# ArtyZe/yolo_quantization

Hardware: AMD Instinct MI355X
Metric: images/sec yolov3-tiny INT8 416x416 (higher is better)
Workload: dtype u8 x s8 -> int32 (f64 or exact-integer requant, bit-identical); 1 GPU; yolov3-tiny full net (cfg/yolov3-tiny_quant.cfg, leaky, per-channel quant), batch 64/GPU synthetic uint8 416x416, inputs resident in HBM (NCHW uint8); global_batch=64, parallelism=image-sharded x1, RCCL weight broadcast once, batches_in_flight=4, kernel_plan=throughput (kernels of which two workgroups share a CU)

## Files before the change

### yolo_quantization_amd/csrc/conv_rows16.hip

```cpp
#include "kargs.h"
#include <type_traits>

#define DBG(bit) (false)
#if defined(MI355_ABLATE)
__device__ long long g_rows16_ts[6][4096];
#define TS(k) do { if (threadIdx.x == 0 && blockIdx.x < 4096) g_rows16_ts[k][blockIdx.x] = wall_clock64(); } while (0)
extern "C" int mi355_debug_read_ts16(long long *host)
{
    return hipMemcpyFromSymbol(host, HIP_SYMBOL(g_rows16_ts), sizeof(long long) * 6 * 4096) == hipSuccess ? 0 : -5;
}
#else
#define TS(k) do { } while (0)
#endif
#define WP_DECL do { } while (0)
#define WP_START() do { } while (0)
#define WP_MARK(k) do { } while (0)
#define WP_FLUSH() do { } while (0)

#define DMA16(gsrc, ldst)                                                                               \
    __builtin_amdgcn_global_load_lds((const __attribute__((address_space(1))) void *)(gsrc),           \
                                     (__attribute__((address_space(3))) void *)(ldst), 16, 0, 0)

template <int KS, int BN> constexpr int ra16_stages() { return KS == 3 ? (BN <= 192 ? 4 : 6) : (BN <= 128 ? 4 : 3); }
template <int KS, int BN> constexpr int rb16_stages() { return KS == 3 ? 2 : ra16_stages<KS, BN>(); }
constexpr int rows16_nb_slots(int BN, int RS, int NW, int KS)
{
    const int wmin = RS * 3 / 4, halo = KS == 3 ? 1 : 0;
    const int rows = (BN - 2 + wmin) / wmin + 1 + (BN - 2 + wmin * wmin) / (wmin * wmin) + 2 * halo;
    return (rows * (RS / 16) + NW - 1) / NW;
}

__device__ __forceinline__ void row16_of_pixel(int n, int H, int W, FastDiv fd_hw, FastDiv fd_w, int &grow, int &x)
{
    const int hw = H * W;
    const int b = fd_div(n, fd_hw);
    const int r = n - b * hw;
    const int y = fd_div(r, fd_w);
    x = r - y * W;
    grow = b * (H + 1) + y + 1;
}

template <int BM, int BN, int WMW, int WNW, int RS, int KS, int NBX = 0>
__global__ __launch_bounds__(64 * WMW * WNW, (BM / WMW > 64 ? 1 : 2)) void conv_rows16_i8_kernel(const ConvArgs a)
{
    constexpr int NW = WMW * WNW, NT = 64 * NW;
    constexpr int TM = BM / WMW, TN = BN / WNW;
    constexpr int MI = TM / 16, NI = TN / 16;
    constexpr int ACH = BM / 16;
    static_assert(KS == 3 && TN % 32 == 0, "3x3 only; pixels are dealt in 32-column sub-tiles (two 16-column tiles each)");
    constexpr int DW = (NW == 8 && KS == 3) ? 4 : NW;
    constexpr int APT = (ACH + DW - 1) / DW;
    constexpr int HALO = (KS == 3) ? 1 : 0;
    constexpr int PIECEB = RS * 16;
    constexpr int CPR = RS / 16;
    constexpr int OSTR = BM + 4;
    constexpr int RA_STAGES = ra16_stages<KS, BN>();
    constexpr int RB_STAGES = rb16_stages<KS, BN>();
    constexpr int NBS = rows16_nb_slots(BN, RS, DW, KS) + NBX;
    constexpr int SPS = (NBS + 3) / 4;
    static_assert(TM % 16 == 0 && TN % 32 == 0, "wave tile: 16-row tiles, 32-column sub-tiles");

    extern __shared__ __attribute__((aligned(16))) char smem[];
    char *ldsB = smem + RA_STAGES * BM * 64;
    const int rowb = a.rowb;
    const int bbytes = a.rows_cap * rowb;
    int *ldsS = reinterpret_cast<int *>(ldsB + RB_STAGES * bbytes);
    double *ldsPM = reinterpret_cast<double *>(smem + a.lds_param_off);
    int *ldsPI = reinterpret_cast<int *>(ldsPM + 3 * BM);
    float *ldsYL = reinterpret_cast<float *>(ldsPI + 2 * BM);

    const int tid = threadIdx.x;
    const int lane = tid & 63;
    const int wave = __builtin_amdgcn_readfirstlane(tid >> 6);
    const int wm = wave / WNW, wn = wave % WNW;
    const int kq = lane >> 4, lj = lane & 15;
    const int dwave = wave & (DW - 1);
    const bool issuer = wave < DW;
    TS(0);

    int logical;
    {
        const int nb = gridDim.x, id = blockIdx.x;
        const int q = nb >> 3, r = nb & 7, xcd = id & 7, idx = id >> 3;
        logical = (xcd < r ? xcd * (q + 1) : r * (q + 1) + (xcd - r) * q) + idx;
    }
    int mtile, ntile;
    {
        const int blk = fd_div(logical, a.fd_ntper);
        const int rem = logical - blk * (a.xcd_mb * a.ntiles_n);
        ntile = fd_div(rem, a.fd_mb);
        mtile = blk * a.xcd_mb + (rem - ntile * a.xcd_mb);
    }
    const int n0 = ntile * a.tile_q + min(ntile, a.tile_r);
    const int n_end = n0 + a.tile_q + (ntile < a.tile_r ? 1 : 0);
    const int W1 = a.W + 1, hw = a.H * a.W;

    int gr0, x0;
    row16_of_pixel(n0, a.H, a.W, a.fd_hw, a.fd_w, gr0, x0);
    int gr1, x1;
    row16_of_pixel(n_end - 1, a.H, a.W, a.fd_hw, a.fd_w, gr1, x1);
    const int grow_first = gr0 - HALO;
    const int nrows = gr1 - gr0 + 1 + 2 * HALO;
    const int ndma = nrows * CPR;

    constexpr int NS = NI;
    int bbase[NS];
#pragma unroll
    for (int ns = 0; ns < NS; ++ns) {
        const int n = n0 + ((ns >> 1) * WNW + wn) * 32 + (ns & 1) * 16 + lj;
        int gr, x;
        row16_of_pixel(n < n_end ? n : n_end - 1, a.H, a.W, a.fd_hw, a.fd_w, gr, x);
        const int prow = gr - grow_first - HALO;
        const int pcol = x + 1 - HALO;
        bbase[ns] = prow * rowb + pcol * 16 + kq * PIECEB;
    }
    const int atab0 = (wm * MI) * 1024 + lane * 16;

    const unsigned lds0 = (unsigned)(size_t)(__attribute__((address_space(3))) char *)smem;
#define DMA_S(ldsdst_u32, sbase_ptr, voff_u32)                                                                   \
    asm volatile("s_mov_b32 m0, %0\n\ts_nop 0\n\tglobal_load_lds_dwordx4 %1, %2" ::"s"(ldsdst_u32), "v"(voff_u32), \
                 "s"(sbase_ptr)                                                                                  \
                 : "memory", "m0")
    constexpr int TAPS = KS * KS;
    const int rot = a.debug & 512 ? 0 : ntile - fd_div(ntile, a.fd_nch) * a.nchunks;
    const int kwrap = a.ksteps;
    int aleft = kwrap - rot * TAPS;
    const int8_t *aptr[APT];
    unsigned adst[APT];
#pragma unroll
    for (int i = 0; i < APT; ++i) {
        const int ch = min(dwave + i * DW, ACH - 1);
        aptr[i] = a.wp + ((size_t)(mtile * ACH + ch) * a.ksteps + (size_t)rot * TAPS) * 1024;
        adst[i] = lds0 + (ch << 10);
    }
    const unsigned lane16 = lane * 16;
    auto issueA_next = [&](unsigned stage_off) {
        if (DW < NW && !issuer) return;
        const bool wrap = --aleft == 0;
#pragma unroll
        for (int i = 0; i < APT; ++i) {
            DMA_S(adst[i] + stage_off, aptr[i], lane16);
            aptr[i] += wrap ? 1024 - (long)kwrap * 1024 : 1024;
        }
        if (wrap) aleft = kwrap;
    };
    const long cell0 = (long)a.in_lead + (long)grow_first * W1 - 1;
    unsigned bvoff[NBS], bdst[NBS];
#pragma unroll
    for (int i = 0; i < NBS; ++i) {
        const int j = min(dwave + i * DW, ndma - 1);
        const int r = j / CPR, cj = j - r * CPR;
        const int o = cj * 1024 + lane * 16;
        const int p = o / PIECEB, c = (o - p * PIECEB) >> 4;
        long f = cell0 + (long)r * W1 + c;
        f = f < 0 ? 0 : (f > a.in_cells - 1 ? a.in_cells - 1 : f);
        bvoff[i] = (unsigned)(f * a.in_cs + p * 16);
        bdst[i] = lds0 + RA_STAGES * BM * 64 + r * rowb + (cj << 10);
    }
    auto issueB_slots = [&](int chunk, auto lo_c, auto hi_c) {
        constexpr int LO = decltype(lo_c)::value, HI = decltype(hi_c)::value;
        if (DW < NW && !issuer) return;
        const unsigned boff = (chunk % RB_STAGES) * bbytes;
        int phys = chunk + rot;
        if (phys >= a.nchunks) phys -= a.nchunks;
        const int8_t *base = a.x + (size_t)phys * 64;
#pragma unroll
        for (int i = LO; i < HI; ++i) {
            const unsigned d = bdst[i] + boff, v = bvoff[i];
            DMA_S(d, base, v);
        }
    };
    auto issueB = [&](int chunk) { issueB_slots(chunk, std::integral_constant<int, 0>{}, std::integral_constant<int, NBS>{}); };

    TS(1);
    if constexpr (KS == 3) {
        issueB(0);
#pragma unroll
        for (int st = 0; st < RA_STAGES - 1; ++st) issueA_next(st * (BM * 64));
    } else {
#pragma unroll
        for (int st = 0; st < RA_STAGES - 1; ++st)
            if (st < a.ksteps) {
                issueB(st);
                issueA_next(st * (BM * 64));
            }
    }

    v4i acc[MI][NI];
#pragma unroll
    for (int mi = 0; mi < MI; ++mi) {
        const int4 c4 = *reinterpret_cast<const int4 *>(a.cwb + mtile * BM + wm * TM + mi * 16 + 4 * kq);
#pragma unroll
        for (int ni = 0; ni < NI; ++ni) acc[mi][ni] = v4i{c4.x, c4.y, c4.z, c4.w};
    }

    for (int i = tid; i < a.rows_cap * RS; i += NT) ldsS[i] = 0;
    if (a.yolo_out)
        for (int i = tid; i < 256; i += NT) ldsYL[i] = yolo_entry_act((float)(i - a.zp_act) * a.s_act, 0);
    for (int i = tid; i < BM; i += NT) {
        const int oc = mtile * BM + i;
        ldsPM[i] = a.mval[oc];
        ldsPM[BM + i] = a.sval[oc];
        ldsPI[i] = a.dzp[oc];
        ldsPI[BM + i] = a.bias[oc];
        ldsPM[2 * BM + i] = a.mprime[oc];
    }

    auto cell_sums = [&](const char *Bt) {
        const int ncells = nrows * RS;
        for (int id = tid; id < ncells; id += NT) {
            const int r = id / RS, c = id - r * RS;
            const char *p0 = Bt + r * rowb + c * 16;
            int t = 0;
#pragma unroll 1
            for (int p = 0; p < 4; ++p) {
                const v4i v = *reinterpret_cast<const v4i *>(p0 + p * PIECEB);
                t = __builtin_amdgcn_sdot4(v[0], 0x01010101, t, false);
                t = __builtin_amdgcn_sdot4(v[1], 0x01010101, t, false);
                t = __builtin_amdgcn_sdot4(v[2], 0x01010101, t, false);
                t = __builtin_amdgcn_sdot4(v[3], 0x01010101, t, false);
            }
            ldsS[id] += t;
        }
    };

    {
        constexpr int R = RA_STAGES;
        static_assert(R >= 4 && R <= 6, "ring depths the stage bookkeeping below is written for");
        static_assert((MI == 4 || MI == 8) && NI >= 2, "written for 64-row wave tiles (128-row ones: one wave per SIMD, accumulators in the AGPRs)");
        constexpr int ROT = 9 % R;
        v4i fa[MI], fb[NI];
        unsigned aaddr[R], baddr[NI];
        unsigned sst[R];
#pragma unroll
        for (int st = 0; st < R; ++st) sst[st] = st * (BM * 64);
#pragma unroll
        for (int st = 0; st < R; ++st) aaddr[st] = lds0 + st * (BM * 64) + atab0;
#pragma unroll
        for (int ni = 0; ni < NI; ++ni) baddr[ni] = lds0 + R * BM * 64 + bbase[ni];
#define LDS_READ128(dst, addr, imm) asm volatile("ds_read_b128 %0, %1 offset:%2" : "=v"(dst) : "v"(addr), "n"(imm))
        using std::integral_constant;
        using std::true_type;
        using std::false_type;
        asm volatile("s_waitcnt vmcnt(%0)" ::"n"((R - 3) * APT) : "memory");
        __builtin_amdgcn_s_barrier();
        TS(2);
#pragma unroll
        for (int ni = 0; ni < NI - 2; ++ni) LDS_READ128(fb[ni], baddr[ni], 0);
#pragma unroll
        for (int mi = 0; mi < MI; ++mi) LDS_READ128(fa[mi], aaddr[0], mi * 1024);
        LDS_READ128(fb[NI - 2], baddr[NI - 2], 0);
        LDS_READ128(fb[NI - 1], baddr[NI - 1], 0);
        auto chunk_body = [&](auto last_c, int chunk) {
            constexpr bool LAST = decltype(last_c)::value;
            const char *Bt = ldsB + (chunk & 1) * bbytes;
            const bool odd = chunk & 1;
            auto step = [&](auto t_c) {
                constexpr int t = decltype(t_c)::value;
                constexpr int TAPN = ((t + 1) % 3) * 16;
                constexpr int SN = (t == 8) ? 0 : (t + 1) % R;
                constexpr bool RD = (t < 8) || !LAST;
                constexpr bool ISSUE_A = !LAST || (t + R - 1 < 9);
                constexpr auto n_b = [](int st) { return (LAST || st < 0 || st >= 4) ? 0 : ((st + 1) * SPS < NBS ? (st + 1) * SPS : NBS) - (st * SPS < NBS ? st * SPS : NBS); };
                constexpr auto n_a = [](int st) { return (st < 0 || !LAST || st + R - 1 < 9) ? APT : 0; };
                constexpr int YOUNG = n_a(t - 1) + n_b(t - 1) + (R > 4 ? n_a(t - 2) + n_b(t - 2) : 0) + (R > 5 ? n_a(t - 3) + n_b(t - 3) : 0);
                constexpr int BLO = t * SPS < NBS ? t * SPS : NBS, BHI = (t + 1) * SPS < NBS ? (t + 1) * SPS : NBS;
                if (t == 8 && !LAST) {
                    const int bdelta = (odd ? -bbytes : bbytes) - 2 * rowb;
                    unsigned rot[R];
#pragma unroll
                    for (int st = 0; st < R; ++st) rot[st] = aaddr[(st + ROT) % R];
#pragma unroll
                    for (int st = 0; st < R; ++st) aaddr[st] = rot[st];
                    if constexpr (R == 5) {
                        unsigned srot[R];
#pragma unroll
                        for (int st = 0; st < R; ++st) srot[st] = sst[(st + ROT) % R];
#pragma unroll
                        for (int st = 0; st < R; ++st) sst[st] = srot[st];
                    }
#pragma unroll
                    for (int ni = 0; ni < NI; ++ni) baddr[ni] += bdelta;
                }
                if (t == 2 || t == 5) {
#pragma unroll
                    for (int ni = 0; ni < NI; ++ni) baddr[ni] += rowb;
                }
                if (t > 0 || chunk > 0) {
                    asm volatile("s_waitcnt vmcnt(%0)" ::"n"(YOUNG) : "memory");
                    __builtin_amdgcn_s_barrier();
                }
                auto dma = [&] {
                    __builtin_amdgcn_sched_barrier(0);
                    if (!LAST && t < 4) issueB_slots(chunk + 1, integral_constant<int, BLO>{}, integral_constant<int, BHI>{});
                    if (ISSUE_A) {
                        if constexpr (R == 6) {
                            constexpr unsigned E = ((t + R - 1) % R) * (BM * 64), O = ((t + R - 1 + 3) % R) * (BM * 64);
                            issueA_next(odd ? O : E);
                        } else if constexpr (R == 5) {
                            issueA_next(sst[t == 8 ? (t + R - 1 - 9) % R : (t + R - 1) % R]);
                        } else {
                            issueA_next((unsigned)((chunk + t + R - 1) & 3) * (BM * 64));
                        }
                    }
                    __builtin_amdgcn_sched_barrier(0);
                };
                asm volatile("s_waitcnt lgkmcnt(2)" ::: "memory");
                __builtin_amdgcn_sched_barrier(0);
#pragma unroll
                for (int ni = 0; ni < NI - 2; ++ni) {
#pragma unroll
                    for (int mi = 0; mi < MI; ++mi) {
                        acc[mi][ni] = __builtin_amdgcn_mfma_i32_16x16x64_i8(fa[mi], fb[ni], acc[mi][ni], 0, 0, 0);
                        if (ni == 0 && mi == 0) dma();
                    }
                    __builtin_amdgcn_sched_barrier(0);
                    if (RD) LDS_READ128(fb[ni], baddr[ni], TAPN);
                    __builtin_amdgcn_sched_barrier(0);
                }
                if (RD) asm volatile("s_waitcnt lgkmcnt(%0)" ::"n"(NI - 2) : "memory");
                else asm volatile("s_waitcnt lgkmcnt(0)" ::: "memory");
                __builtin_amdgcn_sched_barrier(0);
#pragma unroll
                for (int mi = 0; mi < MI; ++mi) {
                    acc[mi][NI - 2] = __builtin_amdgcn_mfma_i32_16x16x64_i8(fa[mi], fb[NI - 2], acc[mi][NI - 2], 0, 0, 0);
                    if (NI == 2 && mi == 0) dma();
                    acc[mi][NI - 1] = __builtin_amdgcn_mfma_i32_16x16x64_i8(fa[mi], fb[NI - 1], acc[mi][NI - 1], 0, 0, 0);
                    __builtin_amdgcn_sched_barrier(0);
                    if (RD) LDS_READ128(fa[mi], aaddr[SN], mi * 1024);
                    __builtin_amdgcn_sched_barrier(0);
                }
                if (RD) {
                    LDS_READ128(fb[NI - 2], baddr[NI - 2], TAPN);
                    LDS_READ128(fb[NI - 1], baddr[NI - 1], TAPN);
                }
                __builtin_amdgcn_sched_barrier(0);
                if (t == 1) {
                    asm volatile("s_waitcnt lgkmcnt(0)" ::: "memory");
                    cell_sums(Bt);
                    asm volatile("s_waitcnt lgkmcnt(0)" ::: "memory");
                    __builtin_amdgcn_sched_barrier(0);
                }
            };
            step(integral_constant<int, 0>{}); step(integral_constant<int, 1>{}); step(integral_constant<int, 2>{});
            step(integral_constant<int, 3>{}); step(integral_constant<int, 4>{}); step(integral_constant<int, 5>{});
            step(integral_constant<int, 6>{}); step(integral_constant<int, 7>{}); step(integral_constant<int, 8>{});
        };
        for (int chunk = 0; chunk + 1 < a.nchunks; ++chunk) chunk_body(false_type{}, chunk);
        chunk_body(true_type{}, a.nchunks - 1);
        asm volatile("s_waitcnt lgkmcnt(0)" ::: "memory");
#undef LDS_READ128
    }

    TS(3);
    if (DBG(32)) {
        if (acc[0][0][0] == 0x7fffffff && a.y) a.y[tid] = 1;
        return;
    }
    __syncthreads();
    int sx[NS];
    bool nvalid[NS];
#pragma unroll
    for (int ns = 0; ns < NS; ++ns) {
        int t = 0;
        const int n = n0 + ((ns >> 1) * WNW + wn) * 32 + (ns & 1) * 16 + lj;
        nvalid[ns] = n < n_end;
        int gr, x;
        row16_of_pixel(nvalid[ns] ? n : n_end - 1, a.H, a.W, a.fd_hw, a.fd_w, gr, x);
        const int c0 = (gr - grow_first - HALO) * RS + x + 1 - HALO;
#pragma unroll
        for (int dy = 0; dy < KS; ++dy)
#pragma unroll
            for (int dx = 0; dx < KS; ++dx) t += ldsS[c0 + dy * RS + dx];
        sx[ns] = t;
    }
    __syncthreads();
    char *otile = smem;
    int *celltab = reinterpret_cast<int *>(smem + BN * OSTR);
    const int m0 = mtile * BM;

    int pb_[NS], rem[NS], nl_[NS];
#pragma unroll
    for (int ns = 0; ns < NS; ++ns) {
        const int nl = ((ns >> 1) * WNW + wn) * 32 + (ns & 1) * 16 + lj;
        nl_[ns] = nl;
        const int nn = nvalid[ns] ? n0 + nl : 0;
        const int b = fd_div(nn, a.fd_hw);
        const int rem0 = nn - b * hw;
        const int y = fd_div(rem0, a.fd_w), xx = rem0 - y * a.W;
        pb_[ns] = b;
        rem[ns] = rem0;
        if (wm == 0 && kq == 0) {
            const int up = a.up;
            celltab[nl] = !nvalid[ns] ? -1
                          : up == 1   ? a.out_lead + (b * (a.H + 1) + (y + 1)) * W1 + xx
                                      : a.out_lead + (b * (up * a.H + 1) + (up * y + 1)) * (up * a.W + 1) + up * xx;
        }
    }
    const bool fast = !a.acc_out && a.hdr->pow2 == 1;
    auto epi_fast = [&](auto act_c, auto sat_c) {
        constexpr int ACT = decltype(act_c)::value;
        constexpr bool SAT = decltype(sat_c)::value != 0;
        constexpr int NH = (NS % 3 == 0) ? 3 : 2;
        static_assert(NS % NH == 0, "pixel tiles per lane");
#pragma unroll
        for (int mi = 0; mi < MI; ++mi) {
            const int ocl = wm * TM + mi * 16 + 4 * kq;
            const int4 dz4 = *reinterpret_cast<const int4 *>(ldsPI + ocl);
            const int dzv[4] = {dz4.x, dz4.y, dz4.z, dz4.w};
            double mp[4];
#pragma unroll
            for (int r = 0; r < 4; ++r) mp[r] = ldsPM[2 * BM + ocl + r];
#pragma unroll
            for (int n0h = 0; n0h < NS; n0h += NH) {
                int32_t accb[4][NH];
#pragma unroll
                for (int r = 0; r < 4; ++r)
#pragma unroll
                    for (int k = 0; k < NH; ++k)
                        accb[r][k] = acc[mi][n0h + k][r] + __mul24(dzv[r], sx[n0h + k]);
                int32_t v[4][NH];
                requant_values<ACT, SAT, NH>(accb, mp, a.zp_act, v);
#pragma unroll
                for (int k = 0; k < NH; ++k)
                    *reinterpret_cast<uint32_t *>(otile + nl_[n0h + k] * OSTR + ocl) = pack4_biased(v[0][k], v[1][k], v[2][k], v[3][k]);
                if (a.y_f32) {
#pragma unroll
                    for (int r = 0; r < 4; ++r) {
                        const int oc = m0 + ocl + r;
                        if (oc < a.n) {
                            const int e = a.yolo_out ? oc % a.yolo_per : 0;
#pragma unroll
                            for (int k = 0; k < NH; ++k)
                                if (nvalid[n0h + k]) {
                                    const int u8 = v[r][k] & 0xFF;
                                    const float f = (float)(u8 - a.zp_act) * a.s_act;
                                    const size_t ridx = ((size_t)pb_[n0h + k] * a.n + oc) * hw + rem[n0h + k];
                                    a.y_f32[ridx] = f;
                                    if (a.yolo_out) a.yolo_out[ridx] = (e == 2 || e == 3) ? f : ldsYL[u8];
                                }
                        }
                    }
                }
            }
        }
    };
    using std::integral_constant;
    if (DBG(64)) {
    } else if (fast) {
#ifdef MI355_EPI_ONE
        epi_fast(integral_constant<int, MI355_ACT_LEAKY>{}, integral_constant<int, 0>{});
    }
    if (false) {
#endif
        const bool sat = a.store_mode == MI355_STORE_SATURATE;
        if (a.act == MI355_ACT_LEAKY) {
            if (sat) epi_fast(integral_constant<int, MI355_ACT_LEAKY>{}, integral_constant<int, 1>{});
            else epi_fast(integral_constant<int, MI355_ACT_LEAKY>{}, integral_constant<int, 0>{});
        } else if (a.act == MI355_ACT_RELU6) {
            if (sat) epi_fast(integral_constant<int, MI355_ACT_RELU6>{}, integral_constant<int, 1>{});
            else epi_fast(integral_constant<int, MI355_ACT_RELU6>{}, integral_constant<int, 0>{});
        } else {
            if (sat) epi_fast(integral_constant<int, MI355_ACT_LINEAR>{}, integral_constant<int, 1>{});
            else epi_fast(integral_constant<int, MI355_ACT_LINEAR>{}, integral_constant<int, 0>{});
        }
    }
#ifndef MI355_EPI_ONE
    else {
#pragma unroll
        for (int mi = 0; mi < MI; ++mi) {
            const int ocl = wm * TM + mi * 16 + 4 * kq;
            const int oc0 = m0 + ocl;
            if (oc0 >= a.n) {
#pragma unroll
                for (int ns = 0; ns < NS; ++ns) *reinterpret_cast<uint32_t *>(otile + nl_[ns] * OSTR + ocl) = 0x80808080u;
                continue;
            }
            uint32_t packed[NS];
#pragma unroll
            for (int ns = 0; ns < NS; ++ns) packed[ns] = 0;
#pragma unroll
            for (int r = 0; r < 4; ++r) {
                const int oc = oc0 + r;
                const int dzv = ldsPI[ocl + r], biv = ldsPI[BM + ocl + r];
                const double mv = ldsPM[ocl + r], sv = ldsPM[BM + ocl + r];
#pragma unroll
                for (int ns = 0; ns < NS; ++ns) {
                    const int32_t accv = acc[mi][ns][r] - biv + dzv * sx[ns];
                    uint32_t u8 = 0;
                    if (oc < a.n) {
                        u8 = requant_u8(accv, biv, mv, sv, a.zp_act, a.act, a.store_mode);
                        if (nvalid[ns] && (a.acc_out || a.y_f32)) {
                            const size_t ridx = ((size_t)pb_[ns] * a.n + oc) * hw + rem[ns];
                            if (a.acc_out) a.acc_out[ridx] = accv;
                            if (a.y_f32) {
                                const float f = (float)((int)u8 - a.zp_act) * a.s_act;
                                a.y_f32[ridx] = f;
                                if (a.yolo_out) {
                                    const int e = oc % a.yolo_per;
                                    a.yolo_out[ridx] = (e == 2 || e == 3) ? f : ldsYL[u8];
                                }
                            }
                        }
                    }
                    packed[ns] |= (u8 ^ 0x80u) << (8 * r);
                }
            }
#pragma unroll
            for (int ns = 0; ns < NS; ++ns) *reinterpret_cast<uint32_t *>(otile + nl_[ns] * OSTR + ocl) = packed[ns];
        }
    }
#endif
    __syncthreads();
    TS(4);
    if (a.y && !DBG(128)) {
        const int dwords = min(BM, a.out_w - m0) >> 2;
        if (a.up > 1) {
            const int total = BN * dwords, rowc = a.up * a.W + 1;
            for (int p = tid; p < total; p += NT) {
                const int pix = p / dwords, d = p - pix * dwords;
                const int cell = celltab[pix];
                if (cell >= 0) {
                    const uint32_t v = *reinterpret_cast<const uint32_t *>(otile + pix * OSTR + d * 4);
                    for (int uy = 0; uy < a.up; ++uy)
                        for (int ux = 0; ux < a.up; ++ux)
                            *reinterpret_cast<uint32_t *>(a.y + (size_t)(cell + uy * rowc + ux) * a.out_cs + m0 + d * 4) = v;
                }
            }
        } else if (dwords == BM / 4 && !(a.out_cs & 15) && !((size_t)a.y & 15)) {
#pragma unroll 2
            for (int p = tid; p < BN * (BM / 16); p += NT) {
                const int pix = p / (BM / 16), q = p % (BM / 16);
                const int cell = celltab[pix];
                if (cell >= 0) {
                    const uint32_t *sp = reinterpret_cast<const uint32_t *>(otile + pix * OSTR + q * 16);
                    const uint4 v = make_uint4(sp[0], sp[1], sp[2], sp[3]);
                    *reinterpret_cast<uint4 *>(a.y + (size_t)cell * a.out_cs + m0 + q * 16) = v;
                }
            }
        } else if (dwords == BM / 4) {
#pragma unroll 4
            for (int p = tid; p < BN * (BM / 4); p += NT) {
                const int pix = p / (BM / 4), d = p % (BM / 4);
                const int cell = celltab[pix];
                if (cell >= 0)
                    *reinterpret_cast<uint32_t *>(a.y + (size_t)cell * a.out_cs + m0 + d * 4) =
                        *reinterpret_cast<const uint32_t *>(otile + pix * OSTR + d * 4);
            }
        } else {
            const int total = BN * dwords;
            for (int p = tid; p < total; p += NT) {
                const int pix = p / dwords, d = p - pix * dwords;
                const int cell = celltab[pix];
                if (cell >= 0)
                    *reinterpret_cast<uint32_t *>(a.y + (size_t)cell * a.out_cs + m0 + d * 4) =
                        *reinterpret_cast<const uint32_t *>(otile + pix * OSTR + d * 4);
            }
        }
    }
    TS(5);
}

template <int BM, int BN, int WMW, int WNW, int RS, int KS, int NBX = 0>
static int rows16_launch_cfg(ConvArgs &a, hipStream_t st)
{
    constexpr int NW = WMW * WNW, NT = 64 * NW;
    constexpr int DW = (NW == 8 && KS == 3) ? 4 : NW;
    constexpr int HALO = (KS == 3) ? 1 : 0;
    if (a.mpad % BM) return MI355_EINVAL;
    a.mtiles = a.mpad / BM;
    if (a.ntiles_n < (a.total_n + BN - 1) / BN) a.ntiles_n = (a.total_n + BN - 1) / BN;
    a.tile_q = a.total_n / a.ntiles_n; a.tile_r = a.total_n % a.ntiles_n;
    {
        const int hw = a.H * a.W;
        auto grow = [&](long n) { const long b = n / hw, r = n - b * hw; return (int)(b * (a.H + 1) + r / a.W + 1); };
        int span = 0;
        for (int t = 0; t < a.ntiles_n; ++t) {
            const long n0 = (long)t * a.tile_q + (t < a.tile_r ? t : a.tile_r), n1 = n0 + a.tile_q + (t < a.tile_r ? 1 : 0) - 1;
            if (n1 < n0) continue;
            const int sp = grow(n1) - grow(n0) + 1;
            if (sp > span) span = sp;
        }
        a.rows_cap = span + 2 * HALO;
    }
    const int ndma = a.rows_cap * (RS / 16);
    if ((ndma + DW - 1) / DW > rows16_nb_slots(BN, RS, DW, KS) + NBX) return MI355_EINVAL;
    if ((size_t)a.in_cells * (size_t)a.in_cs >= ((size_t)1 << 32)) return MI355_EINVAL;
    a.rowb = RS * 64 + 16 * (a.W & 15);
    a.fd_hw = fastdiv_make((uint32_t)(a.H * a.W)); a.fd_w = fastdiv_make((uint32_t)a.W);
    a.fd_ntn = fastdiv_make((uint32_t)a.ntiles_n); a.fd_nch = fastdiv_make((uint32_t)a.nchunks);
    size_t lds = (size_t)ra16_stages<KS, BN>() * BM * 64 + (size_t)rb16_stages<KS, BN>() * a.rows_cap * a.rowb + (size_t)a.rows_cap * RS * 4;
    const size_t lds_epi = (size_t)BN * (BM + 4) + (size_t)BN * 4;
    if (lds_epi > lds) lds = lds_epi;
    lds = (lds + 15) & ~(size_t)15;
    a.lds_param_off = (int)lds;
    lds += (size_t)BM * 32 + (a.yolo_out ? 1024 : 0);
    if (lds > 160 * 1024) return MI355_EINVAL;
    auto kern = conv_rows16_i8_kernel<BM, BN, WMW, WNW, RS, KS, NBX>;
    static size_t lds_attr_dev[64] = {0};
    int dev_ix = 0;
    (void)hipGetDevice(&dev_ix);
    size_t &lds_attr = lds_attr_dev[dev_ix & 63];
    if (lds > 64 * 1024 && lds > lds_attr) {
        lds_attr = lds;
        if (hipFuncSetAttribute(reinterpret_cast<const void *>(kern), hipFuncAttributeMaxDynamicSharedMemorySize,
                                (int)lds) != hipSuccess)
            return MI355_EHIP;
    }
    a.xcd_mb = 1;
    if (!(a.debug & (1 << 24))) {
        const long nb = (long)a.ntiles_n * a.mtiles, per = (nb + 7) / 8;
        const double wslab = (double)BM * a.ksteps * 64, itile = (double)a.total_n / a.ntiles_n * a.cb * a.nchunks;
        double best = 0;
        for (int mb = 1; mb <= a.mtiles; ++mb) {
            if (a.mtiles % mb) continue;
            const long blk = (long)mb * a.ntiles_n;
            const long mt = std::min<long>(a.mtiles, mb * ((per + blk - 1) / blk)), nt = std::min<long>(a.ntiles_n, (per + mb - 1) / mb + (per % mb || blk % per || nb % 8 ? 1 : 0));
            const double bytes = mt * wslab + nt * itile;
            if (mb == 1 || bytes < best) { best = bytes; a.xcd_mb = mb; }
        }
    }
    a.fd_ntper = fastdiv_make((uint32_t)(a.xcd_mb * a.ntiles_n));
    a.fd_mb = fastdiv_make((uint32_t)a.xcd_mb);
    dim3 grid(a.ntiles_n * a.mtiles), block(NT);
    conv_launch_note(grid.x, NT, lds);
    hipLaunchKernelGGL(kern, grid, block, lds, st, a);
    return hipGetLastError() == hipSuccess ? MI355_OK : MI355_EHIP;
}

template <int RS>
static int rows16_launch_tile(ConvArgs &a, hipStream_t st, int bm, int bn)
{
    if (bm == 128 && bn == 384) return rows16_launch_cfg<128, 384, 2, 4, RS, 3>(a, st);
    if (bm == 128 && bn == 256) return rows16_launch_cfg<128, 256, 2, 4, RS, 3>(a, st);
    if (bm == 128 && bn == 192) return rows16_launch_cfg<128, 192, 2, 2, RS, 3>(a, st);
    if (bm == 128 && bn == 128) return rows16_launch_cfg<128, 128, 2, 2, RS, 3>(a, st);
    if (bm == 64 && bn == 256) return rows16_launch_cfg<64, 256, 1, 4, RS, 3>(a, st);
    if (bm == 64 && bn == 128) return rows16_launch_cfg<64, 128, 1, 4, RS, 3>(a, st);
    return MI355_EINVAL;
}

int conv_rows16_launch(ConvArgs &a, hipStream_t st, int bm, int bn)
{
    if (a.cb != 64 || a.ksize != 3) return MI355_EINVAL;
    const int need = a.W + 2;
    if (need <= 16) return rows16_launch_tile<16>(a, st, bm, bn);
    if (need <= 32 && need < 24 && bm == 128 && bn == 384) return rows16_launch_cfg<128, 384, 2, 4, 32, 3, 4>(a, st);
    return MI355_EINVAL;
}
```

Measured before the change: 272,600 images/s.

## Interleave input cell-sum reads into the MFMA K-steps instead of a separate pass

When each thread owns at most one cell (CPT==1), the per-cell byte sums used for zero-point correction are accumulated in registers. Each chunk does one ds_read_b128 plus four sdot4 ops, spread over K-steps 0, 2, 4 and 6 between fragment reads and MFMAs. The sums are written to LDS once after the main loop. This removes the separate cell_sums pass at step 1, its two lgkmcnt(0) drains, and the initial LDS zeroing. In exchange it adds registers and one more outstanding LDS read to the waitcnt bookkeeping. The debug macro is also made live under the ablation build.

```diff
diff --git a/yolo_quantization_amd/csrc/conv_rows16.hip b/yolo_quantization_amd/csrc/conv_rows16.hip
--- a/yolo_quantization_amd/csrc/conv_rows16.hip
+++ b/yolo_quantization_amd/csrc/conv_rows16.hip
@@ -1,8 +1,8 @@
 #include "kargs.h"
 #include <type_traits>
 
-#define DBG(bit) (false)
 #if defined(MI355_ABLATE)
+#define DBG(bit) ((a.debug & (bit)) != 0)
 __device__ long long g_rows16_ts[6][4096];
 #define TS(k) do { if (threadIdx.x == 0 && blockIdx.x < 4096) g_rows16_ts[k][blockIdx.x] = wall_clock64(); } while (0)
 extern "C" int mi355_debug_read_ts16(long long *host)
@@ -10,6 +10,7 @@
     return hipMemcpyFromSymbol(host, HIP_SYMBOL(g_rows16_ts), sizeof(long long) * 6 * 4096) == hipSuccess ? 0 : -5;
 }
 #else
+#define DBG(bit) (false)
 #define TS(k) do { } while (0)
 #endif
 #define WP_DECL do { } while (0)
@@ -59,6 +60,10 @@
     constexpr int NBS = rows16_nb_slots(BN, RS, DW, KS) + NBX;
     constexpr int SPS = (NBS + 3) / 4;
     static_assert(TM % 16 == 0 && TN % 32 == 0, "wave tile: 16-row tiles, 32-column sub-tiles");
+    constexpr int CPT = (NBS * DW * 16 + NT - 1) / NT;
+    static_assert(CPT * NT >= NBS * DW * 16 && CPT >= 1 && CPT <= 2, "a chunk's 4 CPT piece reads ride on its K-steps 0..7, one each");
+    constexpr bool COUNTED = CPT == 1;
+    constexpr auto cs_slot = [](int t) { return !COUNTED ? -1 : CPT == 2 ? (t >= 0 && t < 8 ? t : -1) : (t >= 0 && t < 8 && !(t & 1) ? t >> 1 : -1); };
 
     extern __shared__ __attribute__((aligned(16))) char smem[];
     char *ldsB = smem + RA_STAGES * BM * 64;
@@ -194,7 +199,8 @@
         for (int ni = 0; ni < NI; ++ni) acc[mi][ni] = v4i{c4.x, c4.y, c4.z, c4.w};
     }
 
-    for (int i = tid; i < a.rows_cap * RS; i += NT) ldsS[i] = 0;
+    if constexpr (!COUNTED)
+        for (int i = tid; i < a.rows_cap * RS; i += NT) ldsS[i] = 0;
     if (a.yolo_out)
         for (int i = tid; i < 256; i += NT) ldsYL[i] = yolo_entry_act((float)(i - a.zp_act) * a.s_act, 0);
     for (int i = tid; i < BM; i += NT) {
@@ -239,6 +245,16 @@
 #pragma unroll
         for (int ni = 0; ni < NI; ++ni) baddr[ni] = lds0 + R * BM * 64 + bbase[ni];
 #define LDS_READ128(dst, addr, imm) asm volatile("ds_read_b128 %0, %1 offset:%2" : "=v"(dst) : "v"(addr), "n"(imm))
+        int csum[CPT];
+        unsigned caddr[CPT];
+        v4i cv;
+#pragma unroll
+        for (int k = 0; k < CPT; ++k) {
+            const int id = tid + k * NT, cid = id < nrows * RS ? id : 0;
+            const int r = cid / RS, c = cid - r * RS;
+            caddr[k] = lds0 + R * BM * 64 + r * rowb + c * 16;
+            csum[k] = 0;
+        }
         using std::integral_constant;
         using std::true_type;
         using std::false_type;
@@ -265,7 +281,30 @@
                 constexpr auto n_a = [](int st) { return (st < 0 || !LAST || st + R - 1 < 9) ? APT : 0; };
                 constexpr int YOUNG = n_a(t - 1) + n_b(t - 1) + (R > 4 ? n_a(t - 2) + n_b(t - 2) : 0) + (R > 5 ? n_a(t - 3) + n_b(t - 3) : 0);
                 constexpr int BLO = t * SPS < NBS ? t * SPS : NBS, BHI = (t + 1) * SPS < NBS ? (t + 1) * SPS : NBS;
+                constexpr int CJ = cs_slot(t), DJ = cs_slot(t - 1);
+                static_assert(CJ < 4 * CPT && (CJ < 0 || RD), "cell reads ride on steps that read fragments");
+                auto cell_piece = [&] {
+                    if constexpr (DJ >= 0) {
+                        if (!DBG(16)) {
+                            int s = csum[DJ / 4];
+                            s = __builtin_amdgcn_sdot4(cv[0], 0x01010101, s, false);
+                            s = __builtin_amdgcn_sdot4(cv[1], 0x01010101, s, false);
+                            s = __builtin_amdgcn_sdot4(cv[2], 0x01010101, s, false);
+                            s = __builtin_amdgcn_sdot4(cv[3], 0x01010101, s, false);
+                            csum[DJ / 4] = s;
+                        }
+                        __builtin_amdgcn_sched_barrier(0);
+                    }
+                    if constexpr (CJ >= 0) {
+                        LDS_READ128(cv, caddr[CJ / 4], (CJ % 4) * PIECEB);
+                        __builtin_amdgcn_sched_barrier(0);
+                    }
+                };
                 if (t == 8 && !LAST) {
+                    if constexpr (COUNTED) {
+#pragma unroll
+                        for (int k = 0; k < CPT; ++k) caddr[k] += odd ? -bbytes : bbytes;
+                    }
                     const int bdelta = (odd ? -bbytes : bbytes) - 2 * rowb;
                     unsigned rot[R];
 #pragma unroll
@@ -317,8 +356,9 @@
                     __builtin_amdgcn_sched_barrier(0);
                     if (RD) LDS_READ128(fb[ni], baddr[ni], TAPN);
                     __builtin_amdgcn_sched_barrier(0);
-                }
-                if (RD) asm volatile("s_waitcnt lgkmcnt(%0)" ::"n"(NI - 2) : "memory");
+                    if (ni == 0) cell_piece();
+                }
+                if (RD) asm volatile("s_waitcnt lgkmcnt(%0)" ::"n"(NI - 2 + (NI > 2 && CJ >= 0 ? 1 : 0)) : "memory");
                 else asm volatile("s_waitcnt lgkmcnt(0)" ::: "memory");
                 __builtin_amdgcn_sched_barrier(0);
 #pragma unroll
@@ -329,13 +369,14 @@
                     __builtin_amdgcn_sched_barrier(0);
                     if (RD) LDS_READ128(fa[mi], aaddr[SN], mi * 1024);
                     __builtin_amdgcn_sched_barrier(0);
+                    if (NI == 2 && mi == 0) cell_piece();
                 }
                 if (RD) {
                     LDS_READ128(fb[NI - 2], baddr[NI - 2], TAPN);
                     LDS_READ128(fb[NI - 1], baddr[NI - 1], TAPN);
                 }
                 __builtin_amdgcn_sched_barrier(0);
-                if (t == 1) {
+                if (!COUNTED && t == 1 && !DBG(16)) {
                     asm volatile("s_waitcnt lgkmcnt(0)" ::: "memory");
                     cell_sums(Bt);
                     asm volatile("s_waitcnt lgkmcnt(0)" ::: "memory");
@@ -349,6 +390,11 @@
         for (int chunk = 0; chunk + 1 < a.nchunks; ++chunk) chunk_body(false_type{}, chunk);
         chunk_body(true_type{}, a.nchunks - 1);
         asm volatile("s_waitcnt lgkmcnt(0)" ::: "memory");
+        if constexpr (COUNTED) {
+#pragma unroll
+            for (int k = 0; k < CPT; ++k)
+                if (tid + k * NT < nrows * RS) ldsS[tid + k * NT] = csum[k];
+        }
 #undef LDS_READ128
     }
 
```

New measurement: 275,500 images/s (median of 6 runs). +1.1%, better.
